# ludoplex/llamafile

Measured on AMD Instinct MI355X. Metric: prefill + decode tokens/sec, Llama-3-8B Q4_K_M, 1/2/4/8 MI355X vs CPU tinyBLAS, higher is better.
Workload: dtype int8; 1 GPU; llama3-8b-q4_k_m mat-muls (225 GGML_OP_MUL_MAT per pass, f32 activations in, quantisation fused, sibling ops fused at decode), 512-token prefill + 128 decode, matmul-only; model=llama3-8b-q4_k_m, parallelism=single GPU, hip_graph=True, weight_bytes_per_gpu=4616331264, decode_launches_per_pass=129

## Files before the change

### llamafile_amd/csrc/gemv_common.h

```cpp
#pragma once
#include "lfamd_device.h"
#include "gemv_launch.h"

__device__ static inline void load_piece(float (&v)[16], const float *x, int p) {
    const float4 *src = (const float4 *)(x + (size_t)p * 16);
#pragma unroll
    for (int e = 0; e < 4; e++) {
        float4 f = src[e];
        v[4 * e + 0] = f.x, v[4 * e + 1] = f.y, v[4 * e + 2] = f.z, v[4 * e + 3] = f.w;
    }
}

template <bool K, int N>
__device__ static inline void pack_codes(uint32_t (&y)[N / 4], const float (&v)[N], float scale) {
#pragma unroll
    for (int e = 0; e < N; e++) {
        int q;
        if constexpr (K) {
            q = (int)rintf(scale * v[e]);
            q = q > 127 ? 127 : q;
        } else {
            q = (int)roundf(v[e] * scale);
        }
        y[e >> 2] |= (uint32_t)(q & 0xff) << (8 * (e & 3));
    }
}

__device__ __forceinline__ void x80_quantise_piece(uint8_t *lds, int nquads, const float (&v)[16], int c, int p) {
    float amax = 0.0f;
#pragma unroll
    for (int e = 0; e < 16; e++)
        amax = fmaxf(amax, fabsf(v[e]));
    amax = fmaxf(amax, __shfl_xor(amax, 1, 64));
    const float d = amax / 127.0f;
    const float id = d != 0.0f ? 1.0f / d : 0.0f;
    uint32_t y[4] = {0, 0, 0, 0};
    pack_codes<false>(y, v, id);
    const int l = p >> 1, hf = p & 1;
    uint8_t *dst = lds + (size_t)(c * nquads + (l >> 2)) * X80_QUAD + (l & 3) * 4;
#pragma unroll
    for (int e = 0; e < 4; e++)
        *(uint32_t *)(dst + (4 * hf + e) * 16) = y[e];
    if (hf == 0)
        *(float *)(dst + X80_QD) = h2f(f2h_bits(d));
}
__device__ __forceinline__ void x80_copy_blocks(uint8_t *lds, int nquads, const uint8_t *__restrict__ B, size_t b_row_bytes, long col0, int nc,
                                                int nblocks, int nthr) {
    for (int idx = threadIdx.x; idx < nc * nblocks * 9; idx += nthr) {
        int c = idx / (nblocks * 9), rem = idx % (nblocks * 9);
        int l = rem / 9, w = rem % 9;
        const uint8_t *y = B + (col0 + c) * b_row_bytes + (size_t)l * 34;
        uint32_t v;
        if (w < 8) {
            const uint16_t *p = (const uint16_t *)(y + 2 + 4 * w);
            v = (uint32_t)p[0] | ((uint32_t)p[1] << 16);
        } else {
            v = __builtin_bit_cast(uint32_t, h2f(*(const uint16_t *)y));
        }
        *(uint32_t *)(lds + (size_t)(c * nquads + (l >> 2)) * X80_QUAD + (l & 3) * 4 + (w < 8 ? w * 16 : X80_QD)) = v;
    }
}

#ifndef GEMV_DIAG
#define GEMV_DIAG 0
#endif
#if GEMV_DIAG
#ifndef GEMV_DIAG_WG
#define GEMV_DIAG_WG 100
#endif
#define DIAG_STAMPS (4 * 16 * 16)
#include "diag_stamps.h"
static __device__ unsigned long long g_gemv_wg[512 * 4];
extern "C" __attribute__((weak)) int lfamd_debug_gemv_wgs(unsigned long long *dst) {
    return (int)hipMemcpyFromSymbol(dst, HIP_SYMBOL(g_gemv_wg), sizeof(g_gemv_wg));
}
#define GWG(slot)                                                                                                \
    do {                                                                                                         \
        if (blockIdx.x < 512 && threadIdx.x == 0) {                                                              \
            g_gemv_wg[blockIdx.x * 4 + (slot)] = __builtin_amdgcn_s_memrealtime();                               \
            if ((slot) == 0) {                                                                                   \
                g_gemv_wg[blockIdx.x * 4 + 2] = (unsigned long long)__builtin_amdgcn_s_getreg(4 | (31 << 11)) |  \
                                                ((unsigned long long)__builtin_amdgcn_s_getreg(20 | (31 << 11)) << 32); \
                gwg_clk0 = __builtin_amdgcn_s_memtime();                                                         \
            } else {  \
                g_gemv_wg[blockIdx.x * 4 + 3] = __builtin_amdgcn_s_memtime() - gwg_clk0;                         \
            }                                                                                                    \
        }                                                                                                        \
    } while (0)
#define GSTAMP()                                                                                                 \
    do {                                                                                                         \
        __builtin_amdgcn_sched_barrier(0);                                                                       \
        if ((blockIdx.x == 0 || blockIdx.x == GEMV_DIAG_WG) && lane == 0 && stamp_n < 16)                                  \
            g_stamps[((blockIdx.x ? 1 : 0) * 16 + wave) * 16 + stamp_n++] = DIAG_REALTIME();                      \
        __builtin_amdgcn_sched_barrier(0);                                                                       \
    } while (0)
#define GSTAMP_ARRIVAL()                                                                                         \
    do {                                                                                                         \
        asm volatile("s_waitcnt vmcnt(0)" ::: "memory");                                                         \
        GSTAMP();                                                                                                \
    } while (0)
#else
#define GSTAMP()
#define GSTAMP_ARRIVAL()
#define GWG(slot)
#endif
```

### llamafile_amd/csrc/gemv_impl.h

```cpp
#pragma once
#include "gemv_common.h"


__device__ static inline int put_group(uint8_t *dst, int grp, uint32_t y0, uint32_t y1) {
    const uint32_t p0 = __builtin_amdgcn_perm(y1, y0, 0x05010400);
    const uint32_t p1 = __builtin_amdgcn_perm(y1, y0, 0x07030602);
    const int pos = (grp & 16) | ((grp & 1) << 3) | ((grp & 8) >> 1) | ((grp >> 1) & 3);
    *(uint2 *)(dst + 8 * pos) = make_uint2(p0, p1);
    int hs = sdot4(y0, 0x01010101u, 0);
    hs = sdot4(y1, 0x01010101u, hs);
    *(int16_t *)(dst + XBLK_HB + 2 * pos) = (int16_t)hs;
    return hs;
}

__device__ static inline void put_pair(uint8_t *dst, int grp, int hs_even_plus_odd) {
    const int pp = ((grp & 16) >> 1) | ((grp & 1) << 2) | ((grp & 8) >> 2) | ((grp >> 2) & 1);
    *(int16_t *)(dst + XBLK_PS + 2 * pp) = (int16_t)hs_even_plus_odd;
}

__device__ static inline int put_group_pair(uint8_t *dst, int grp, uint32_t y0, uint32_t y1) {
    const int hs = put_group(dst, grp, y0, y1);
    const int pair = hs + (int)dpp_u32<DPP_XOR2>((uint32_t)hs);
    if ((grp & 2) == 0)
        put_pair(dst, grp, pair);
// ... 420 lines not shown
    struct chunk {
        uint4 q0[GEMV_CH_MAX], q1[GEMV_CH_MAX];
        uint2 hd[GEMV_CH_MAX], hm[GEMV_CH_MAX], hq[GEMV_CH_MAX];
    };
    __device__ static inline void load(chunk &ch, int s, lfamd_rsrc r, uint32_t off, int gsel, int slot, int hrow) {
        ch.q0[s] = buf_ld16_nt(r, off + (2 * gsel + 0) * 1024 + slot * 16);
        ch.q1[s] = buf_ld16_nt(r, off + (2 * gsel + 1) * 1024 + slot * 16);
        ch.hd[s] = buf_ld8(r, off + PCL_D + hrow * 16 + gsel * 8);
        if constexpr (HAS_M)
            ch.hm[s] = buf_ld8(r, off + PCL_M + hrow * 16 + gsel * 8);
        if constexpr (HAS_H)
            ch.hq[s] = buf_ld8(r, off + PCL_QH + slot * 16 + gsel * 8);
    }
    __device__ static inline float dot(const chunk &ch, int s, const uint8_t *xb, int gsel, int h) {
        const uint4 q0 = ch.q0[s], q1 = ch.q1[s];
        const uint2 hd = ch.hd[s];
        const kq_words8 qw = kq_words_of(q0, q1);
        const kq_codes y = kq_codes_of(xb, gsel, h);
        const uint4 dsw = *(const uint4 *)(xb + XBLK_D + 16 * gsel);
        const uint32_t dsv[4] = {dsw.x, dsw.y, dsw.z, dsw.w};
        kq_sums4 ps = {};
        if constexpr (!HAS_M)
            ps = kq_pair_sums_of(xb, gsel, h);
        float acc = 0.0f;
#pragma unroll
        for (int jj = 0; jj < 4; jj++) {
            int isum = 0;
#pragma unroll
            for (int d2 = 0; d2 < 2; d2++) {
                const int t8 = 2 * jj + d2;
                const uint32_t x = qw.w[t8];
                uint32_t c0 = x & 0x0F0F0F0F, c1 = (x >> 4) & 0x0F0F0F0F;
                if constexpr (HAS_H) {
                    const uint32_t Hd = (t8 < 4 ? ch.hq[s].x : ch.hq[s].y) >> (t8 & 3);
                    c0 |= Hd & 0x10101010;
                    c1 |= ((Hd >> 4) & 0x00100010) | ((Hd << 12) & 0x10001000);
                }
                isum = sdot4(c0, y.w[2 * t8], isum);
                isum = sdot4(c1, y.w[2 * t8 + 1], isum);
            }
            const float d = kq_h4(hd, jj);
            if constexpr (HAS_M) {
                const float m = kq_h4(ch.hm[s], jj);
                const float d8 = h2f((uint16_t)(dsv[jj] & 0xffff)), s8 = h2f((uint16_t)(dsv[jj] >> 16));
                acc = fmaf(d * d8, (float)isum, acc);
                acc = fmaf(m, h ? 0.0f : s8, acc);
            } else {
                acc = fmaf(d * __builtin_bit_cast(float, dsv[jj]), (float)(isum - 16 * ps.v[jj]), acc);
            }
        }
        return acc;
    }
};

template <int TYPE>
struct pk_traits {
    static constexpr int ACT = LFAMD_TYPE_Q8_K;
    static constexpr bool Q3 = TYPE == LFAMD_TYPE_Q3_K;
    static constexpr int TILE = Q3 ? PK3_TILE : PK2_TILE;
    static constexpr bool MINS = !Q3;
    static constexpr int OFF = Q3 ? 4 : 0;
    struct chunk {
        uint4 q[GEMV_CH_MAX];
        uint2 hb[GEMV_CH_MAX], sc[GEMV_CH_MAX];
        uint32_t dd[GEMV_CH_MAX];
    };
    __device__ static inline void load(chunk &ch, int s, lfamd_rsrc r, uint32_t off, int gsel, int slot, int hrow) {
        ch.q[s] = buf_ld16_nt(r, off + gsel * 1024 + slot * 16);
        if constexpr (Q3)
            ch.hb[s] = buf_ld8(r, off + PK3_HB + gsel * 512 + slot * 8);
        ch.sc[s] = buf_ld8(r, off + (Q3 ? PK3_SC : PK2_SC) + hrow * 16 + gsel * 8);
        ch.dd[s] = __builtin_amdgcn_raw_buffer_load_b32(r, off + (Q3 ? PK3_D : PK2_D) + hrow * 4, 0, 0);
    }
    __device__ static inline float dot(const chunk &ch, int s, const uint8_t *xb, int gsel, int h) {
        const uint4 qc = ch.q[s];
        const uint2 scb = ch.sc[s];
        const uint32_t dw = ch.dd[s];
        const float d = h2f((uint16_t)(dw & 0xffff));
        const uint32_t cw[4] = {qc.x, qc.y, qc.z, qc.w};
        const kq_codes y = kq_codes_of(xb, gsel, h);
        const kq_words4 hbv = kq_group_sums_of(xb, gsel, h);
        int sumi = 0, summ = 0;
#pragma unroll
        for (int t8 = 0; t8 < 8; t8++) {
            uint32_t x = ((t8 & 1) ? (cw[t8 >> 1] >> 2) : cw[t8 >> 1]) & 0x33333333u;
            if constexpr (Q3) {
                const uint32_t H = (t8 < 4 ? ch.hb[s].x : ch.hb[s].y) >> (t8 & 3);
                x |= (H & 0x11111111u) << 2;
            }
            const int isum = kq_nib_dot(x, y, t8, 0);
            const int hs = (int)(int16_t)((hbv.w[t8 >> 1] >> (16 * (t8 & 1))) & 0xffff);
            const uint32_t sbyte = ((t8 < 4 ? scb.x : scb.y) >> (8 * (t8 & 3))) & 0xff;
            if constexpr (Q3) {
                sumi += (int)(int8_t)sbyte * (isum - OFF * hs);
            } else {
                sumi += (int)(sbyte & 15) * isum;
                summ += (int)(sbyte >> 4) * hs;
            }
        }
        const float d8 = *(const float *)(xb + XBLK_D);
        if constexpr (MINS)
            return fmaf(d * d8, (float)sumi, -(h2f((uint16_t)(dw >> 16)) * d8) * (float)summ);
        return (d * d8) * (float)sumi;
    }
};

struct iq4c_traits {
    static constexpr int ACT = LFAMD_TYPE_Q8_K;
    static constexpr int TILE = P4K_TILE;
    struct chunk {
        uint4 q0[GEMV_CH_MAX], q1[GEMV_CH_MAX], hd[GEMV_CH_MAX];
    };
    __device__ static inline void load(chunk &ch, int s, lfamd_rsrc r, uint32_t off, int gsel, int slot, int hrow) {
        ch.q0[s] = buf_ld16_nt(r, off + (2 * gsel + 0) * 1024 + slot * 16);
        ch.q1[s] = buf_ld16_nt(r, off + (2 * gsel + 1) * 1024 + slot * 16);
        ch.hd[s] = buf_ld16(r, off + P4K_HDR + hrow * 16);
    }
    __device__ static inline float dot(const chunk &ch, int s, const uint8_t *xb, int gsel, int h) {
        const uint4 q0 = ch.q0[s], q1 = ch.q1[s], hd = ch.hd[s];
        const kq_words8 qw = kq_words_of(q0, q1);
        const kq_codes y = kq_codes_of(xb, gsel, h);
        const uint32_t scw = gsel ? hd.y : hd.x;
        int sumi = 0;
#pragma unroll
        for (int u = 0; u < 4; u++) {
            int isum = 0;
#pragma unroll
            for (int e = 0; e < 2; e++) {
                isum = kq_nib_dot<true>(qw.w[2 * u + e], y, 2 * u + e, isum);
            }
            sumi += (int)(int8_t)((scw >> (8 * u)) & 0xff) * isum;
        }
        const float d8 = *(const float *)(xb + XBLK_D);
        return (h2f((uint16_t)(hd.z & 0xffff)) * d8) * (float)sumi;
    }
};



__device__ static inline void put_codes_wave(uint8_t *dst, uint32_t y, int lane) {
    const int hf = lane & 1, grp = lane >> 1;
    const uint32_t other = dpp_u32<DPP_XOR1>(y);
    const uint32_t lo = hf ? other : y, hi = hf ? y : other;
    const uint32_t word = hf ? __builtin_amdgcn_perm(hi, lo, 0x07030602) : __builtin_amdgcn_perm(hi, lo, 0x05010400);
    const int pos = (grp & 16) | ((grp & 1) << 3) | ((grp & 8) >> 1) | ((grp >> 1) & 3);
    *(uint32_t *)(dst + 8 * pos + 4 * hf) = word;
    const int s4 = sdot4(y, 0x01010101u, 0);
    const int hs = s4 + (int)dpp_u32<DPP_XOR1>((uint32_t)s4);
    if (hf == 0)
        *(int16_t *)(dst + XBLK_HB + 2 * pos) = (int16_t)hs;
    const int hs2 = hs + (int)dpp_u32<DPP_ROW_SHL4>((uint32_t)hs);
    if ((lane & 5) == 0)
        put_pair(dst, grp, hs2);
}

__device__ static inline void stage_f32_q8k_wave(uint8_t *dst, const float4 v, int lane) {
    const float a0 = fabsf(v.x), a1 = fabsf(v.y), a2 = fabsf(v.z), a3 = fabsf(v.w);
    float am = fmaxf(fmaxf(a0, a1), fmaxf(a2, a3));
    am = fmaxf(am, dpp_f32<DPP_XOR1>(am));
    am = fmaxf(am, dpp_f32<DPP_XOR2>(am));
    am = fmaxf(am, dpp_f32<DPP_HALF_MIRROR>(am));
    am = fmaxf(am, dpp_f32<DPP_MIRROR>(am));
    const float amax = fmaxf(fmaxf(readlane_f32(am, 0), readlane_f32(am, 16)), fmaxf(readlane_f32(am, 32), readlane_f32(am, 48)));
    const bool m0 = a0 == amax, m1 = a1 == amax, m2 = a2 == amax, m3 = a3 == amax;
    const unsigned long long ball = __builtin_amdgcn_ballot_w64(m0 || m1 || m2 || m3);
    const float cand = m0 ? v.x : (m1 ? v.y : (m2 ? v.z : v.w));
    const int first = ball ? __builtin_ctzll(ball) : 0;
    const bool nz = amax != 0.0f;
    const float val = nz ? readlane_f32(cand, first) : 1.0f;
    const float iscale = -128.0f / val;
    int q0 = (int)rintf(iscale * v.x), q1 = (int)rintf(iscale * v.y), q2 = (int)rintf(iscale * v.z), q3 = (int)rintf(iscale * v.w);
    q0 = q0 > 127 ? 127 : q0, q1 = q1 > 127 ? 127 : q1, q2 = q2 > 127 ? 127 : q2, q3 = q3 > 127 ? 127 : q3;
    uint32_t y = (uint32_t)(q0 & 0xff) | ((uint32_t)(q1 & 0xff) << 8) | ((uint32_t)(q2 & 0xff) << 16) | ((uint32_t)(q3 & 0xff) << 24);
    y = nz ? y : 0u;
    const float d = nz ? 1.0f / iscale : 0.0f;
    put_codes_wave(dst, y, lane);
    if (lane == 0)
        *(float *)(dst + XBLK_D) = d;
}

template <bool S1>
__device__ static inline void stage_f32_q80_wave(uint8_t *dst, const float4 v, int lane) {
    float am = fmaxf(fmaxf(fabsf(v.x), fabsf(v.y)), fmaxf(fabsf(v.z), fabsf(v.w)));
    am = fmaxf(am, dpp_f32<DPP_XOR1>(am));
    am = fmaxf(am, dpp_f32<DPP_XOR2>(am));
    am = fmaxf(am, dpp_f32<DPP_HALF_MIRROR>(am));
    const float d = am / 127.0f;
    const float id = d != 0.0f ? 1.0f / d : 0.0f;
    const int q0 = (int)roundf(v.x * id), q1 = (int)roundf(v.y * id), q2 = (int)roundf(v.z * id), q3 = (int)roundf(v.w * id);
    const uint32_t y = (uint32_t)(q0 & 0xff) | ((uint32_t)(q1 & 0xff) << 8) | ((uint32_t)(q2 & 0xff) << 16) | ((uint32_t)(q3 & 0xff) << 24);
    put_codes_wave(dst, y, lane);
    int sum = 0;
    if constexpr (S1) {
        sum = sdot4(y, 0x01010101u, 0);
        sum += (int)dpp_u32<DPP_XOR1>((uint32_t)sum);
        sum += (int)dpp_u32<DPP_XOR2>((uint32_t)sum);
        sum += (int)dpp_u32<DPP_HALF_MIRROR>((uint32_t)sum);
    }
    if ((lane & 7) == 0)
        put_scale_q80<S1>(dst, lane >> 3, d, sum);
}

__device__ static inline void stage_f32_q8k_wave2(uint8_t *dst, const float4 va, const float4 vb, int lane) {
    const float v[8] = {va.x, va.y, va.z, va.w, vb.x, vb.y, vb.z, vb.w};
    float a[8];
#pragma unroll
    for (int e = 0; e < 8; e++)
        a[e] = fabsf(v[e]);
    float am = fmaxf(fmaxf(fmaxf(a[0], a[1]), fmaxf(a[2], a[3])), fmaxf(fmaxf(a[4], a[5]), fmaxf(a[6], a[7])));
    am = fmaxf(am, dpp_f32<DPP_XOR1>(am));
    am = fmaxf(am, dpp_f32<DPP_XOR2>(am));
    am = fmaxf(am, dpp_f32<DPP_HALF_MIRROR>(am));
    am = fmaxf(am, dpp_f32<DPP_MIRROR>(am));
    const bool hi = lane >= 32;
    const float amax_lo = fmaxf(readlane_f32(am, 0), readlane_f32(am, 16)), amax_hi = fmaxf(readlane_f32(am, 32), readlane_f32(am, 48));
    const float amax = hi ? amax_hi : amax_lo;
    bool any = false;
    float cand = v[7];
#pragma unroll
    for (int e = 7; e >= 0; e--) {
        const bool me = a[e] == amax;
        cand = me ? v[e] : cand;
        any = any || me;
    }
    const unsigned long long ball = __builtin_amdgcn_ballot_w64(any);
    const uint32_t blo = (uint32_t)ball, bhi = (uint32_t)(ball >> 32);
    const int first_lo = blo ? __builtin_ctz(blo) : 0, first_hi = 32 + (bhi ? __builtin_ctz(bhi) : 0);
    const float val_lo = readlane_f32(cand, first_lo), val_hi = readlane_f32(cand, first_hi);
    const bool nz = amax != 0.0f;
    const float val = nz ? (hi ? val_hi : val_lo) : 1.0f;
    const float iscale = -128.0f / val;
    uint32_t y[2] = {0, 0};
    pack_codes<true>(y, v, iscale);
    const uint32_t y0 = nz ? y[0] : 0u, y1 = nz ? y[1] : 0u;
    const float d = nz ? 1.0f / iscale : 0.0f;
    const int grp = lane & 31;
    put_group_pair(dst, grp, y0, y1);
    if (grp == 0)
        *(float *)(dst + XBLK_D) = d;
}

template <bool S1>
__device__ static inline void stage_f32_q80_wave2(uint8_t *dst, const float4 va, const float4 vb, int lane) {
    const float v[8] = {va.x, va.y, va.z, va.w, vb.x, vb.y, vb.z, vb.w};
    float am = 0.0f;
#pragma unroll
    for (int e = 0; e < 8; e++)
        am = fmaxf(am, fabsf(v[e]));
    am = fmaxf(am, dpp_f32<DPP_XOR1>(am));
    am = fmaxf(am, dpp_f32<DPP_XOR2>(am));
    const float d = am / 127.0f;
    const float id = d != 0.0f ? 1.0f / d : 0.0f;
    uint32_t y[2] = {0, 0};
    pack_codes<false>(y, v, id);
    const int grp = lane & 31;
    const int pair = put_group_pair(dst, grp, y[0], y[1]);
    const int sum = pair + (int)dpp_u32<DPP_XOR1>((uint32_t)pair);
    if ((grp & 3) == 0)
        put_scale_q80<S1>(dst, grp >> 2, d, sum);
}

template <int ACT, bool TAIL = false>
__device__ static inline void stage_quantised_wave(uint8_t *dst, const uint8_t *row_generic, int b, int lane, int kb = 0) {
    typedef const __attribute__((address_space(1))) uint8_t *gptr;
    const gptr row = (gptr)row_generic;
    if (lane < 32) {
        const int grp = lane;
        uint32_t y0, y1;
        if constexpr (ACT == LFAMD_TYPE_Q8_K) {
            const gptr y = row + (size_t)b * 292;
            const __attribute__((address_space(1))) uint32_t *src = (const __attribute__((address_space(1))) uint32_t *)(y + 36 + 8 * grp);
            y0 = src[0], y1 = src[1];
            if (grp == 0)
                *(float *)(dst + XBLK_D) = *(const __attribute__((address_space(1))) float *)y;
        } else {
            constexpr bool S1 = ACT == LFAMD_TYPE_Q8_1;
            const gptr blk = row + (size_t)(b * 8 + (grp >> 2)) * (S1 ? 36 : 34);
            const bool in = !TAIL || b * 8 + (grp >> 2) < kb;
            y0 = y1 = 0;
            if (in) {
                const __attribute__((address_space(1))) uint16_t *src = (const __attribute__((address_space(1))) uint16_t *)(blk + (S1 ? 4 : 2) + 8 * (grp & 3));
                y0 = (uint32_t)src[0] | ((uint32_t)src[1] << 16), y1 = (uint32_t)src[2] | ((uint32_t)src[3] << 16);
            }
            if ((grp & 3) == 0) {
                const __attribute__((address_space(1))) uint16_t *hdr = (const __attribute__((address_space(1))) uint16_t *)blk;
                if constexpr (S1)
                    *(uint32_t *)(dst + XBLK_D + 4 * (grp >> 2)) = in ? (uint32_t)hdr[0] | ((uint32_t)hdr[1] << 16) : 0u;
                else
                    *(float *)(dst + XBLK_D + 4 * (grp >> 2)) = in ? h2f(hdr[0]) : 0.0f;
            }
        }
        put_group_pair(dst, grp, y0, y1);
    }
}

#define KQ_F4(u) make_float4(__builtin_bit_cast(float, (u).x), __builtin_bit_cast(float, (u).y), __builtin_bit_cast(float, (u).z), \
                           __builtin_bit_cast(float, (u).w))

template <typename TR>
__device__ __forceinline__ int kq_nb_of(int nbk) {
    if constexpr (TR::ACT == LFAMD_TYPE_Q8_K)
        return nbk;
    else
        return (nbk + 7) >> 3;
}
template <typename TR>
__device__ __forceinline__ uint32_t kq_row_bytes_f32(int nbk) {
    return (uint32_t)nbk * (TR::ACT == LFAMD_TYPE_Q8_K ? 1024u : 128u);
}

template <typename TR, int NC, int BT, int NW, int GEMV_CH, bool IDS>
__device__ __forceinline__ void gemv_kq_body(const gemv_mats &mats, const int nbk, const uint8_t *__restrict__ B, size_t b_row_bytes,
                                             long col0, int n_ht, const int bid, const int gdim, uint8_t *lds) {
    const int nb = kq_nb_of<TR>(nbk), kb = nbk;
    const int lane = threadIdx.x & 63, wave = threadIdx.x >> 6;
    const int i16 = lane & 15, h = (lane >> 4) & 1, gsel = lane >> 5;
    const kq_lds lay = kq_lds_of(NC, nb, NW, 16);
    float *red = (float *)(lds + lay.red);
#if GEMV_DIAG
    int stamp_n = 0;
#endif
    GSTAMP();

    const int sb_per_wave = (nb + NW - 1) / NW;
    const int cpt = (sb_per_wave + GEMV_CH - 1) / GEMV_CH;
    const int ntile = (n_ht - bid + gdim - 1) / gdim;
    const int total = ntile * cpt;

    const int wave_u = __builtin_amdgcn_readfirstlane(wave);
    const uint32_t rt_bytes = (uint32_t)nb * TR::TILE;
    auto mat_of = [&](long ht) __attribute__((always_inline)) {
        int j = 0;
#pragma unroll
        for (int jj = 1; jj < GEMV_MAX_MATS; jj++)
            if (jj < mats.count && ht >= mats.ht_end[jj - 1])
                j = jj;
        return j;
    };
    auto issue = [&](typename TR::chunk &ch, int f) {
        const int tile_i = f / cpt, chunk_i = f - tile_i * cpt;
        long ht = (long)bid + (long)tile_i * gdim;
        const int j = mat_of(ht);
        const uint8_t *A = mats.A[j];
        bool have = f < total;
        if constexpr (IDS) {
            const int ex = mats.ids[mats.id_idx[j]];
            const bool ok = ex >= 0 && ex < mats.experts;
            A += (size_t)(ok ? ex : 0) * mats.expert_bytes;
            have = have && ok;
        }
        if (j > 0)
            ht -= mats.ht_end[j - 1];
        const int hh = (int)(ht & 1);
        const lfamd_rsrc r = make_rsrc(A + (size_t)(ht >> 1) * rt_bytes, have ? rt_bytes : 0u);
        const int slot = h * 32 + hh * 16 + i16, hrow = hh * 16 + i16;
#pragma unroll
        for (int s = 0; s < GEMV_CH; s++) {
            const int b = wave_u + NW * (chunk_i * GEMV_CH + s);
            TR::load(ch, s, r, (uint32_t)b * TR::TILE, gsel, slot, hrow);
        }
    };

    float acc[NC];
#pragma unroll
    for (int c = 0; c < NC; c++)
        acc[c] = 0.0f;

    auto consume = [&](const typename TR::chunk &ch, int f) {
        const int tile_i = f / cpt, chunk_i = f - tile_i * cpt;
#pragma unroll
        for (int s = 0; s < GEMV_CH; s++) {
            const int b = wave + NW * (chunk_i * GEMV_CH + s);
            const int bc = b < nb ? b : nb - 1;
#pragma unroll
            for (int c = 0; c < NC; c++) {
                acc[c] += TR::dot(ch, s, lds + (size_t)(c * nb + bc) * XBLK, gsel, h);
            }
        }
        if (chunk_i == cpt - 1) {
            float *rb = red + (tile_i & 1) * (NW * NC * 16);
#pragma unroll
            for (int c = 0; c < NC; c++) {
                float v = acc[c];
                v += __shfl_xor(v, 16, 64);
                v += __shfl_xor(v, 32, 64);
                if (lane < 16)
                    rb[(wave * NC + c) * 16 + lane] = v;
                acc[c] = 0.0f;
            }
            GSTAMP();
            __syncthreads();
            GSTAMP();
            if (threadIdx.x < 16 * NC) {
                const int c = threadIdx.x >> 4, i = threadIdx.x & 15;
                float v = 0.0f;
#pragma unroll
                for (int w = 0; w < NW; w++)
                    v += rb[(w * NC + c) * 16 + i];
                long ht = (long)bid + (long)tile_i * gdim;
                const int j = mat_of(ht);
                if (j > 0)
                    ht -= mats.ht_end[j - 1];
                const long row = (ht >> 1) * 32 + (ht & 1) * 16 + i;
// ... 148 lines not shown
struct kq_pre {
    const uint8_t *A0, *A1, *A2;
    int e0, e1;
};

template <typename TR, int BT, int NW, int GEMV_CH, bool IDS, bool EARLY = false, bool PAIR = false>
__device__ __forceinline__ void gemv_kq_body1(const gemv_mats &mats, int nbk, const uint8_t *__restrict__ B,
                                              size_t b_row_bytes, long col0, int n_ht, const int bid, int gdim,
                                              uint8_t *lds, const kq_pre pre) {
    if constexpr (EARLY)
        asm volatile("" : "+s"(nbk), "+s"(B), "+s"(n_ht), "+s"(gdim));
    else
        asm volatile("" : "+s"(nbk), "+s"(B), "+s"(b_row_bytes), "+s"(col0), "+s"(n_ht), "+s"(gdim));
    const int nb = kq_nb_of<TR>(nbk), kb = nbk;
    const int lane = threadIdx.x & 63;
    const int wave = __builtin_amdgcn_readfirstlane((int)(threadIdx.x >> 6));
    const int i16 = lane & 15, h = (lane >> 4) & 1, gsel = lane >> 5;
    constexpr int RW = PAIR ? 32 : 16;
    const kq_lds lay = kq_lds_of(1, nb, NW, RW);
    float *red = (float *)(lds + lay.red);
#if GEMV_DIAG
    int stamp_n = 0;
    unsigned long long gwg_clk0 = 0;
#endif
    GWG(0);
    GSTAMP();
    constexpr int JX = GEMV_CH == 1 ? 1 : (NW == 8 ? 2 : 4);
    const uint8_t *xrow = B + col0 * b_row_bytes;
    const lfamd_rsrc rx = make_rsrc(xrow, kq_row_bytes_f32<TR>(nbk));
    uint4 xv[JX];
    auto x_off = [&](int j0, int j) __attribute__((always_inline)) {
        if constexpr (JX == 1)
            return (uint32_t)(wave + NW * j0) * 1024u + (uint32_t)lane * 16u;
        else
            return (uint32_t)(wave + NW * (j0 + 2 * (j >> 1) + (lane >> 5))) * 1024u + (uint32_t)(lane & 31) * 32u + 16u * (j & 1);
    };
    if constexpr (BT == LFAMD_TYPE_F32) {
#pragma unroll
        for (int j = 0; j < JX; j++)
            xv[j] = buf_ld16(rx, x_off(0, j));
        __builtin_amdgcn_sched_barrier(0);
    }
    constexpr bool PRE1 = BT == LFAMD_TYPE_Q8_K && TR::ACT == LFAMD_TYPE_Q8_K && JX <= 2;
    uint2 pq = make_uint2(0, 0);
    uint32_t pd = 0;
    const int pre_b = JX == 1 ? wave : wave + NW * (lane >> 5);
    if constexpr (PRE1) {
        const lfamd_rsrc rq = make_rsrc(xrow, (uint32_t)nb * 292u);
        pq = buf_ld8(rq, (uint32_t)pre_b * 292u + 36u + (uint32_t)(lane & 31) * 8u);
        pd = __builtin_amdgcn_raw_buffer_load_b32(rq, (uint32_t)pre_b * 292u, 0, 0);
        __builtin_amdgcn_sched_barrier(0);
    }
    typename TR::chunk bufA, bufB;
    typename TR::chunk bufA2, bufB2;
    static_assert(!(PAIR && (EARLY || IDS)), "the paired item is a variant of the plain launch");
    constexpr bool early = EARLY && !IDS;
    constexpr bool XPAIR = !PAIR && TR::TILE % 128 != 0;
    auto ht_of = [&](int q) __attribute__((always_inline)) {
        return (XPAIR && q < (n_ht & ~15)) ? ((q & ~15) | ((q & 7) << 1) | ((q >> 3) & 1)) : q;
    };
    if constexpr (early) {
        const int hb = ht_of(bid);
        const bool s1 = hb >= pre.e0, s2 = hb >= pre.e1;
        const uint8_t *Ap = s2 ? pre.A2 : (s1 ? pre.A1 : pre.A0);
        const int hl = hb - (s2 ? pre.e1 : (s1 ? pre.e0 : 0));
        const int hh = hl & 1;
        const uint32_t rtb = (uint32_t)nb * TR::TILE;
        const lfamd_rsrc r = make_rsrc(Ap + (size_t)(hl >> 1) * rtb, hb < n_ht ? rtb : 0u);
#pragma unroll
        for (int s = 0; s < GEMV_CH; s++)
            TR::load(bufA, s, r, (uint32_t)(wave + NW * s) * TR::TILE, gsel, h * 32 + hh * 16 + i16, hh * 16 + i16);
        __builtin_amdgcn_sched_barrier(0);
        GSTAMP();
    }
    const kq_tab tab = kq_table(mats);

    const int sb_per_wave = (nb + NW - 1) / NW;
    const int cpt = (sb_per_wave + GEMV_CH - 1) / GEMV_CH;
    const uint32_t rt_bytes = (uint32_t)nb * TR::TILE;

    float acc = 0.0f, acc2 = 0.0f;
    int par = 0;
    constexpr int HT_STEP = PAIR ? 2 : 1;
    kq_cursor ci{HT_STEP * bid, 0}, cc{HT_STEP * bid, 0};
#define KQ_ADVANCE(c)                                                                                                  \
    do {                                                                                                               \
        if (++(c).chunk == cpt)                                                                                        \
            (c).chunk = 0, (c).ht += HT_STEP * gdim;                                                                   \
    } while (0)
#define KQ_ISSUE(buf)                                                                                                  \
    do {                                                                                                               \
        kq_issue<TR, NW, GEMV_CH, IDS>(buf, mats, tab, kq_cursor{ht_of(ci.ht), ci.chunk}, n_ht, rt_bytes, wave, i16, h, gsel); \
        if constexpr (PAIR) {                                                                                          \
            const kq_cursor c2{ci.ht + 1, ci.chunk};                                                                   \
            kq_issue<TR, NW, GEMV_CH, IDS>(buf##2, mats, tab, c2, n_ht, rt_bytes, wave, i16, h, gsel);                 \
        }                                                                                                              \
        KQ_ADVANCE(ci);                                                                                                \
    } while (0)
#define KQ_CONSUME(buf)                                                                                                \
    do {                                                                                                               \
        GSTAMP_ARRIVAL();                                                                                              \
        _Pragma("unroll") for (int s = 0; s < GEMV_CH; s++) {                                                          \
            const int b = wave + NW * (cc.chunk * GEMV_CH + s);                                                        \
                                                                        \
            if (b < nb) {                                                                                              \
                acc += TR::dot(buf, s, lds + (size_t)b * XBLK, gsel, h);                                               \
                if constexpr (PAIR)                                                                                    \
                    acc2 += TR::dot(buf##2, s, lds + (size_t)b * XBLK, gsel, h);                                       \
            }                                                                                                          \
        }                                                                                                              \
        if (cc.chunk == cpt - 1) {                                                                                     \
            float *rb = red + par * (NW * RW);                                                                         \
            par ^= 1;                                                                                                  \
            float v = kq_sum_rows(acc);                                   \
            if (lane < 16)                                                                                             \
                rb[wave * RW + lane] = v;                                                                              \
            acc = 0.0f;                                                                                                \
            if constexpr (PAIR) {                                                                                      \
                float v2 = kq_sum_rows(acc2);                                                                          \
                if (lane < 16)                                                                                         \
                    rb[wave * RW + 16 + lane] = v2;                                                                    \
                acc2 = 0.0f;                                                                                           \
            }                                                                                                          \
            GSTAMP();                                                                                                  \
            __syncthreads();                                                                                           \
            GSTAMP();                                                                                                  \
            if (threadIdx.x < RW) {                                                                                    \
                const int i = threadIdx.x;                                                                             \
                float t = 0.0f;                                                                                        \
                _Pragma("unroll") for (int w = 0; w < NW; w++) t += rb[w * RW + i];                                    \
                const kq_sel p = kq_pick(tab, ht_of(cc.ht));                                                           \
                const long row = (long)(p.ht >> 1) * 32 + (p.ht & 1) * 16 + i;          \
                bool ok = true;                                                                                        \
                if constexpr (IDS) {                    \
                    const int ex = mats.ids[p.idx];                                                                    \
                    ok = ex >= 0 && ex < mats.experts;                                                                 \
                }                                                                                                      \
                if (row < p.m && ok)                                                                                   \
                    ((__attribute__((address_space(1))) float *)p.C)[col0 * p.ldc + row] = t;                                                                      \
            }                                                                                                          \
        }                                                                                                              \
        KQ_ADVANCE(cc);                                                                                                \
    } while (0)

    if constexpr (BT == LFAMD_TYPE_F32) {
        uint8_t *dummy = (uint8_t *)(red + (lay.dummy - lay.red) / sizeof(float)) + (size_t)wave * XBLK;
        if constexpr (early)
            KQ_ADVANCE(ci);
        else
            KQ_ISSUE(bufA);
        __builtin_amdgcn_sched_barrier(0);
        GSTAMP();
#define KQ_STAGE_GROUP(j0)                                                                                             \
    if constexpr (JX == 1) {                                                                                           \
        const int b = wave + NW * (j0);                                                                                \
        uint8_t *dst = b < nb ? lds + (size_t)b * XBLK : dummy;                                                        \
        if constexpr (TR::ACT == LFAMD_TYPE_Q8_K)                                                                      \
            stage_f32_q8k_wave(dst, KQ_F4(xv[0]), lane);                                                               \
        else                                                                                                           \
            stage_f32_q80_wave<TR::ACT == LFAMD_TYPE_Q8_1>(dst, KQ_F4(xv[0]), lane);                                   \
    } else {                                                                                                           \
        _Pragma("unroll") for (int ps = 0; ps < JX / 2; ps++) {                                                        \
            const int b = wave + NW * ((j0) + 2 * ps + (lane >> 5));                                                   \
            uint8_t *dst = b < nb ? lds + (size_t)b * XBLK : dummy;                                                    \
            if constexpr (TR::ACT == LFAMD_TYPE_Q8_K)                                                                  \
                stage_f32_q8k_wave2(dst, KQ_F4(xv[2 * ps]), KQ_F4(xv[2 * ps + 1]), lane);                              \
            else                                                                                                       \
                stage_f32_q80_wave2<TR::ACT == LFAMD_TYPE_Q8_1>(dst, KQ_F4(xv[2 * ps]), KQ_F4(xv[2 * ps + 1]), lane);  \
        }                                                                                                              \
    }
        KQ_STAGE_GROUP(0)
        for (int j0 = JX; j0 < sb_per_wave; j0 += JX) {
#pragma unroll
            for (int j = 0; j < JX; j++)
                xv[j] = buf_ld16(rx, x_off(j0, j));
            KQ_STAGE_GROUP(j0)
        }
#undef KQ_STAGE_GROUP
    } else {
        if constexpr (early)
            KQ_ADVANCE(ci);
        else
            KQ_ISSUE(bufA);
        GSTAMP();
        if constexpr (PRE1 && JX == 1) {
            if (wave < nb && lane < 32) {
                uint8_t *dst = lds + (size_t)wave * XBLK;
                put_group_pair(dst, lane, pq.x, pq.y);
                if (lane == 0)
                    *(uint32_t *)(dst + XBLK_D) = pd;
            }
        } else if constexpr (PRE1) {
            {
                uint8_t *dummy = (uint8_t *)(red + (lay.dummy - lay.red) / sizeof(float)) + (size_t)wave * XBLK;
                uint8_t *dst = pre_b < nb ? lds + (size_t)pre_b * XBLK : dummy;
                const int grp = lane & 31;
                put_group_pair(dst, grp, pq.x, pq.y);
                if (grp == 0)
                    *(uint32_t *)(dst + XBLK_D) = pd;
            }
            for (int b = wave + 2 * NW; b < nb; b += NW)
                stage_quantised_wave<TR::ACT>(lds + (size_t)b * XBLK, xrow, b, lane);
        } else {
            if (TR::ACT != LFAMD_TYPE_Q8_K && kb != 8 * nb) {
                for (int b = wave; b < nb; b += NW) {
                    if (b * 8 + 8 > kb)
                        stage_quantised_wave<TR::ACT, true>(lds + (size_t)b * XBLK, xrow, b, lane, kb);
                    else
                        stage_quantised_wave<TR::ACT>(lds + (size_t)b * XBLK, xrow, b, lane);
                }
            } else {
                for (int b = wave; b < nb; b += NW)
                    stage_quantised_wave<TR::ACT>(lds + (size_t)b * XBLK, xrow, b, lane);
            }
        }
    }
    __builtin_amdgcn_fence(__ATOMIC_RELEASE, "wavefront");
    GSTAMP();

    for (;;) {
        kq_cursor cn = cc;
        KQ_ADVANCE(cn);
        if (cn.ht >= n_ht)
            break;
        KQ_ISSUE(bufB);
        KQ_CONSUME(bufA);
        GSTAMP();
        KQ_ISSUE(bufA);
        KQ_CONSUME(bufB);
    }
    if (cc.ht < n_ht)
        KQ_CONSUME(bufA);
    GWG(1);
#undef KQ_ADVANCE
#undef KQ_ISSUE
#undef KQ_CONSUME
}

template <typename TR, int NC, int BT, int NW, int GEMV_CH, bool IDS = false, bool PAIR = false>
__global__ __launch_bounds__(NW * 64) void gemv_kq_kernel(const uint8_t *__restrict__ B, size_t b_row_bytes, long col0, int nbk,
                                                          int n_ht, int gdim, const gemv_mats mats) {
    extern __shared__ __attribute__((aligned(16))) uint8_t lds[];
    if constexpr (NC == 1)
        gemv_kq_body1<TR, BT, NW, GEMV_CH, IDS, false, PAIR>(mats, nbk, B, b_row_bytes, col0, n_ht, (int)blockIdx.x, gdim, lds, kq_pre{});
    else
        gemv_kq_body<TR, NC, BT, NW, GEMV_CH, IDS>(mats, nbk, B, b_row_bytes, col0, n_ht, (int)blockIdx.x, gdim, lds);
}

template <typename TR, int NC, int BT, int NW, int GEMV_CH>
__global__ __launch_bounds__(NW * 64) void gemv_kq_early_kernel(const uint8_t *__restrict__ xrow, const uint8_t *__restrict__ A0,
                                                                const uint8_t *__restrict__ A1, const uint8_t *__restrict__ A2, int nbk,
                                                                int n_ht, int gdim, int e0, int e1, const gemv_mats mats) {
    extern __shared__ __attribute__((aligned(16))) uint8_t lds[];
    static_assert(NC == 1, "one activation row (the parameter keeps the kernel's name in line with gemv_kq_kernel's)");
    asm volatile("" : "+s"(A0), "+s"(A1), "+s"(A2), "+s"(e0), "+s"(e1));
    gemv_kq_body1<TR, BT, NW, GEMV_CH, false, true>(mats, nbk, xrow, 0, 0, n_ht, (int)blockIdx.x, gdim, lds, kq_pre{A0, A1, A2, e0, e1});
}

template <typename TR, int BT, int NW, int GEMV_CH>
__global__ __launch_bounds__(NW * 64) void gemv_kq_ids_pair_kernel(const uint8_t *__restrict__ Ba, const uint8_t *__restrict__ Bb,
                                                                   size_t b_row_bytes, int nbk, int n_ht_a, int n_ht_b, int grid_a, int grid_b,
                                                                   const gemv_mats mats_a, const gemv_mats mats_b) {
    extern __shared__ __attribute__((aligned(16))) uint8_t lds[];
    if ((int)blockIdx.x < grid_a)
        gemv_kq_body1<TR, BT, NW, GEMV_CH, true>(mats_a, nbk, Ba, b_row_bytes, 0, n_ht_a, (int)blockIdx.x, grid_a, lds, kq_pre{});
    else
        gemv_kq_body1<TR, BT, NW, GEMV_CH, true>(mats_b, nbk, Bb, b_row_bytes, 0, n_ht_b, (int)blockIdx.x - grid_a, grid_b, lds, kq_pre{});
}

template <typename TRA, typename TRB, int BT, int NW, int GEMV_CH>
__global__ __launch_bounds__(NW * 64) void gemv_kq_dual_kernel(const uint8_t *__restrict__ B, size_t b_row_bytes, int nbk, int n_ht_a,
                                                               int n_ht_b, int grid_a, int grid_b, const gemv_mats mats_a,
                                                               const gemv_mats mats_b) {
    extern __shared__ __attribute__((aligned(16))) uint8_t lds[];
    static_assert(TRA::ACT == TRB::ACT, "both types must share the activation image, and so the meaning of nbk (kq_nb_of)");
    if ((int)blockIdx.x < grid_a)
        gemv_kq_body1<TRA, BT, NW, GEMV_CH, false>(mats_a, nbk, B, b_row_bytes, 0, n_ht_a, (int)blockIdx.x, grid_a, lds, kq_pre{});
    else
        gemv_kq_body1<TRB, BT, NW, GEMV_CH, false>(mats_b, nbk, B, b_row_bytes, 0, n_ht_b, (int)blockIdx.x - grid_a, grid_b, lds, kq_pre{});
}

template <typename TRA, typename TRB, int BT, int NW, int GEMV_CH>
__global__ __launch_bounds__(NW * 64) void gemv_kq_dual_early_kernel(const uint8_t *__restrict__ xrow, const uint8_t *__restrict__ Aa0,
                                                                     const uint8_t *__restrict__ Aa1, const uint8_t *__restrict__ Ab0, int nbk,
                                                                     int n_ht_a, int n_ht_b, int grid_a, int ea0, int grid_b,
                                                                     const gemv_mats mats_a, const gemv_mats mats_b) {
    extern __shared__ __attribute__((aligned(16))) uint8_t lds[];
    static_assert(TRA::ACT == TRB::ACT, "both types must share the activation image, and so the meaning of nbk (kq_nb_of)");
    asm volatile("" : "+s"(Aa0), "+s"(Aa1), "+s"(Ab0), "+s"(ea0), "+s"(grid_a));
    if ((int)blockIdx.x < grid_a)
        gemv_kq_body1<TRA, BT, NW, GEMV_CH, false, true>(mats_a, nbk, xrow, 0, 0, n_ht_a, (int)blockIdx.x, grid_a, lds,
                                                         kq_pre{Aa0, Aa1, Aa1, ea0, KQ_NO_BOUNDARY});
    else
        gemv_kq_body1<TRB, BT, NW, GEMV_CH, false, true>(mats_b, nbk, xrow, 0, 0, n_ht_b, (int)blockIdx.x - grid_a, grid_b, lds,
                                                         kq_pre{Ab0, Ab0, Ab0, KQ_NO_BOUNDARY, KQ_NO_BOUNDARY});
}


template <typename TR, int BT, bool ROWS32>
static const void *kq_kernel_1(int variant, int nw, int ch) {
    const int form = nw * 10 + ch;
    if (variant == LFAMD_GEMV_PLAIN)
        return form == 82    ? (const void *)gemv_kq_kernel<TR, 1, BT, 8, 2>
               : form == 161 ? (const void *)gemv_kq_kernel<TR, 1, BT, 16, 1>
               : form == 162 ? (const void *)gemv_kq_kernel<TR, 1, BT, 16, 2>
                             : nullptr;
    if (variant == LFAMD_GEMV_EARLY)
        return form == 82    ? (const void *)gemv_kq_early_kernel<TR, 1, BT, 8, 2>
               : form == 161 ? (const void *)gemv_kq_early_kernel<TR, 1, BT, 16, 1>
               : form == 162 ? (const void *)gemv_kq_early_kernel<TR, 1, BT, 16, 2>
                             : nullptr;
    if constexpr (ROWS32)
        if (variant == LFAMD_GEMV_ROWS32 && form == 161)
            return (const void *)gemv_kq_kernel<TR, 1, BT, 16, 1, false, true>;
    return nullptr;
}

template <typename TR, int BT, int NC>
static const void *kq_kernel_n(int nw, int ch) {
    const int form = nw * 10 + ch;
    return form == 161  ? (const void *)gemv_kq_kernel<TR, NC, BT, 16, 1>
           : form == 82 ? (const void *)gemv_kq_kernel<TR, NC, BT, 8, 2>
           : form == 84 ? (const void *)gemv_kq_kernel<TR, NC, BT, 8, 4>
                        : nullptr;
}

template <typename TR, int BT, bool ROWS32>
static const void *kq_kernel(int variant, int nc, int nw, int ch) {
    static const void *(*const cols[])(int, int) = {kq_kernel_n<TR, BT, 2>, kq_kernel_n<TR, BT, 3>, kq_kernel_n<TR, BT, 4>, kq_kernel_n<TR, BT, 5>,
// ... 47 lines not shown
```

Before: 4456 tokens/s.

## Interleave f32 activation staging with weight-chunk pipeline and cheapen quantisation math

Replaces float abs-max reductions with integer-bit max via v_max3 and integer DPP compares, and replaces per-element int conversion and shift packing with a magic-number rounding trick plus byte permutes. The JX>1 f32 staging path is restructured so that activation loads and quantisation passes alternate with weight-buffer issue/consume steps (double buffering bufA/bufB) instead of staging everything up front. It also makes the diagnostic vmcnt wait conditional. The aim is to overlap activation quantisation with weight streaming and shorten the ALU path. In exchange the control flow is more complex, it adds an early-return path, and it relies on assumptions about chunk layout (GEMV_CH==2).

```diff
diff --git a/llamafile_amd/csrc/gemv_common.h b/llamafile_amd/csrc/gemv_common.h
--- a/llamafile_amd/csrc/gemv_common.h
+++ b/llamafile_amd/csrc/gemv_common.h
@@ -11,18 +11,23 @@
     }
 }
 
+#define KQ_ROUND_MAGIC 12582912.0f
 template <bool K, int N>
 __device__ static inline void pack_codes(uint32_t (&y)[N / 4], const float (&v)[N], float scale) {
+    uint32_t t[N];
 #pragma unroll
     for (int e = 0; e < N; e++) {
-        int q;
-        if constexpr (K) {
-            q = (int)rintf(scale * v[e]);
-            q = q > 127 ? 127 : q;
-        } else {
-            q = (int)roundf(v[e] * scale);
-        }
-        y[e >> 2] |= (uint32_t)(q & 0xff) << (8 * (e & 3));
+        float r;
+        if constexpr (K)
+            r = fminf(scale * v[e] + KQ_ROUND_MAGIC, KQ_ROUND_MAGIC + 127.0f);
+        else
+            r = roundf(v[e] * scale) + KQ_ROUND_MAGIC;
+        t[e] = __builtin_bit_cast(uint32_t, r);
+    }
+#pragma unroll
+    for (int e = 0; e < N; e += 4) {
+        const uint32_t lo = __builtin_amdgcn_perm(t[e + 1], t[e], 0x0c0c0400), hi = __builtin_amdgcn_perm(t[e + 3], t[e + 2], 0x0c0c0400);
+        y[e >> 2] |= __builtin_amdgcn_perm(hi, lo, 0x05040100);
     }
 }
 
@@ -96,7 +101,8 @@
     } while (0)
 #define GSTAMP_ARRIVAL()                                                                                         \
     do {                                                                                                         \
-        asm volatile("s_waitcnt vmcnt(0)" ::: "memory");                                                         \
+        if (GEMV_DIAG >= 2)                                                                                      \
+            asm volatile("s_waitcnt vmcnt(0)" ::: "memory");                                                     \
         GSTAMP();                                                                                                \
     } while (0)
 #else
diff --git a/llamafile_amd/csrc/gemv_impl.h b/llamafile_amd/csrc/gemv_impl.h
--- a/llamafile_amd/csrc/gemv_impl.h
+++ b/llamafile_amd/csrc/gemv_impl.h
@@ -596,6 +596,20 @@
     const int hs2 = hs + (int)dpp_u32<DPP_ROW_SHL4>((uint32_t)hs);
     if ((lane & 5) == 0)
         put_pair(dst, grp, hs2);
+}
+
+__device__ static inline uint32_t kq_absmax8_bits(const float (&v)[8]) {
+    float p, q, r;
+    asm("v_max3_f32 %0, |%1|, |%2|, |%3|" : "=v"(p) : "v"(v[0]), "v"(v[1]), "v"(v[2]));
+    asm("v_max3_f32 %0, |%1|, |%2|, |%3|" : "=v"(q) : "v"(v[3]), "v"(v[4]), "v"(v[5]));
+    asm("v_max3_f32 %0, |%1|, |%2|, %3" : "=v"(r) : "v"(v[6]), "v"(v[7]), "v"(p));
+    const uint32_t qb = __builtin_bit_cast(uint32_t, q), rb = __builtin_bit_cast(uint32_t, r);
+    return qb > rb ? qb : rb;
+}
+template <int CTRL>
+__device__ static inline uint32_t kq_max_dpp(uint32_t x) {
+    const uint32_t o = dpp_u32<CTRL>(x);
+    return o > x ? o : x;
 }
 
 __device__ static inline void stage_f32_q8k_wave(uint8_t *dst, const float4 v, int lane) {
@@ -647,31 +661,26 @@
 
 __device__ static inline void stage_f32_q8k_wave2(uint8_t *dst, const float4 va, const float4 vb, int lane) {
     const float v[8] = {va.x, va.y, va.z, va.w, vb.x, vb.y, vb.z, vb.w};
-    float a[8];
-#pragma unroll
-    for (int e = 0; e < 8; e++)
-        a[e] = fabsf(v[e]);
-    float am = fmaxf(fmaxf(fmaxf(a[0], a[1]), fmaxf(a[2], a[3])), fmaxf(fmaxf(a[4], a[5]), fmaxf(a[6], a[7])));
-    am = fmaxf(am, dpp_f32<DPP_XOR1>(am));
-    am = fmaxf(am, dpp_f32<DPP_XOR2>(am));
-    am = fmaxf(am, dpp_f32<DPP_HALF_MIRROR>(am));
-    am = fmaxf(am, dpp_f32<DPP_MIRROR>(am));
+    const uint32_t lm = kq_absmax8_bits(v);
+    uint32_t am = kq_max_dpp<DPP_XOR1>(lm);
+    am = kq_max_dpp<DPP_XOR2>(am);
+    am = kq_max_dpp<DPP_HALF_MIRROR>(am);
+    am = kq_max_dpp<DPP_MIRROR>(am);
     const bool hi = lane >= 32;
-    const float amax_lo = fmaxf(readlane_f32(am, 0), readlane_f32(am, 16)), amax_hi = fmaxf(readlane_f32(am, 32), readlane_f32(am, 48));
-    const float amax = hi ? amax_hi : amax_lo;
-    bool any = false;
+    const uint32_t r0 = (uint32_t)__builtin_amdgcn_readlane((int)am, 0), r1 = (uint32_t)__builtin_amdgcn_readlane((int)am, 16);
+    const uint32_t r2 = (uint32_t)__builtin_amdgcn_readlane((int)am, 32), r3 = (uint32_t)__builtin_amdgcn_readlane((int)am, 48);
+    const uint32_t amax_lo = r0 > r1 ? r0 : r1, amax_hi = r2 > r3 ? r2 : r3;
+    const uint32_t amax_b = hi ? amax_hi : amax_lo;
+    const float amax = __builtin_bit_cast(float, amax_b);
     float cand = v[7];
 #pragma unroll
-    for (int e = 7; e >= 0; e--) {
-        const bool me = a[e] == amax;
-        cand = me ? v[e] : cand;
-        any = any || me;
-    }
-    const unsigned long long ball = __builtin_amdgcn_ballot_w64(any);
-    const uint32_t blo = (uint32_t)ball, bhi = (uint32_t)(ball >> 32);
-    const int first_lo = blo ? __builtin_ctz(blo) : 0, first_hi = 32 + (bhi ? __builtin_ctz(bhi) : 0);
+    for (int e = 6; e >= 0; e--)
+        cand = fabsf(v[e]) == amax ? v[e] : cand;
+    const unsigned long long ball = __builtin_amdgcn_ballot_w64(lm == amax_b);
+    const uint32_t blo = (uint32_t)ball | 0x80000000u, bhi = (uint32_t)(ball >> 32) | 0x80000000u;
+    const int first_lo = __builtin_ctz(blo), first_hi = 32 + __builtin_ctz(bhi);
     const float val_lo = readlane_f32(cand, first_lo), val_hi = readlane_f32(cand, first_hi);
-    const bool nz = amax != 0.0f;
+    const bool nz = amax_b != 0u;
     const float val = nz ? (hi ? val_hi : val_lo) : 1.0f;
     const float iscale = -128.0f / val;
     uint32_t y[2] = {0, 0};
@@ -687,12 +696,10 @@
 template <bool S1>
 __device__ static inline void stage_f32_q80_wave2(uint8_t *dst, const float4 va, const float4 vb, int lane) {
     const float v[8] = {va.x, va.y, va.z, va.w, vb.x, vb.y, vb.z, vb.w};
-    float am = 0.0f;
-#pragma unroll
-    for (int e = 0; e < 8; e++)
-        am = fmaxf(am, fabsf(v[e]));
-    am = fmaxf(am, dpp_f32<DPP_XOR1>(am));
-    am = fmaxf(am, dpp_f32<DPP_XOR2>(am));
+    uint32_t amb = kq_absmax8_bits(v);
+    amb = kq_max_dpp<DPP_XOR1>(amb);
+    amb = kq_max_dpp<DPP_XOR2>(amb);
+    const float am = __builtin_bit_cast(float, amb);
     const float d = am / 127.0f;
     const float id = d != 0.0f ? 1.0f / d : 0.0f;
     uint32_t y[2] = {0, 0};
@@ -1147,29 +1154,69 @@
         __builtin_amdgcn_sched_barrier(0);
         GSTAMP();
 #define KQ_STAGE_GROUP(j0)                                                                                             \
-    if constexpr (JX == 1) {                                                                                           \
+    {                                                                                                                  \
         const int b = wave + NW * (j0);                                                                                \
         uint8_t *dst = b < nb ? lds + (size_t)b * XBLK : dummy;                                                        \
         if constexpr (TR::ACT == LFAMD_TYPE_Q8_K)                                                                      \
             stage_f32_q8k_wave(dst, KQ_F4(xv[0]), lane);                                                               \
         else                                                                                                           \
             stage_f32_q80_wave<TR::ACT == LFAMD_TYPE_Q8_1>(dst, KQ_F4(xv[0]), lane);                                   \
-    } else {                                                                                                           \
-        _Pragma("unroll") for (int ps = 0; ps < JX / 2; ps++) {                                                        \
-            const int b = wave + NW * ((j0) + 2 * ps + (lane >> 5));                                                   \
-            uint8_t *dst = b < nb ? lds + (size_t)b * XBLK : dummy;                                                    \
-            if constexpr (TR::ACT == LFAMD_TYPE_Q8_K)                                                                  \
-                stage_f32_q8k_wave2(dst, KQ_F4(xv[2 * ps]), KQ_F4(xv[2 * ps + 1]), lane);                              \
-            else                                                                                                       \
-                stage_f32_q80_wave2<TR::ACT == LFAMD_TYPE_Q8_1>(dst, KQ_F4(xv[2 * ps]), KQ_F4(xv[2 * ps + 1]), lane);  \
-        }                                                                                                              \
-    }
-        KQ_STAGE_GROUP(0)
-        for (int j0 = JX; j0 < sb_per_wave; j0 += JX) {
-#pragma unroll
-            for (int j = 0; j < JX; j++)
-                xv[j] = buf_ld16(rx, x_off(j0, j));
-            KQ_STAGE_GROUP(j0)
+    }
+        if constexpr (JX == 1) {
+            KQ_STAGE_GROUP(0)
+            for (int j0 = JX; j0 < sb_per_wave; j0 += JX) {
+                xv[0] = buf_ld16(rx, x_off(j0, 0));
+                KQ_STAGE_GROUP(j0)
+            }
+        } else {
+            static_assert(GEMV_CH == 2 && (JX == 2 || JX == 4), "a pass of two blocks is a chunk of two slots");
+#define KQ_LOAD_PASS(s0, xa, xb)                                                                                       \
+    do {                                                                                                               \
+        const uint32_t o = (uint32_t)(wave + NW * ((s0) + (lane >> 5))) * 1024u + (uint32_t)(lane & 31) * 32u;         \
+        xa = buf_ld16(rx, o), xb = buf_ld16(rx, o + 16u);                                                              \
+    } while (0)
+#define KQ_STAGE_PASS(s0, xa, xb)                                                                                      \
+    do {                                                                                                               \
+        const int b = wave + NW * ((s0) + (lane >> 5));                                                                \
+        uint8_t *dst = b < nb ? lds + (size_t)b * XBLK : dummy;                                                        \
+        if constexpr (TR::ACT == LFAMD_TYPE_Q8_K)                                                                      \
+            stage_f32_q8k_wave2(dst, KQ_F4(xa), KQ_F4(xb), lane);                                                      \
+        else                                                                                                           \
+            stage_f32_q80_wave2<TR::ACT == LFAMD_TYPE_Q8_1>(dst, KQ_F4(xa), KQ_F4(xb), lane);                          \
+        __builtin_amdgcn_fence(__ATOMIC_RELEASE, "wavefront");             \
+        GSTAMP();                                                                                                      \
+    } while (0)
+            constexpr int X1 = JX == 4 ? 2 : 0;
+            KQ_STAGE_PASS(0, xv[0], xv[1]);
+            if (cpt > 1) {
+                if constexpr (JX == 2)
+                    KQ_LOAD_PASS(2, xv[0], xv[1]);
+                KQ_ISSUE(bufB);
+                GSTAMP();
+                KQ_CONSUME(bufA);
+                KQ_STAGE_PASS(2, xv[X1], xv[X1 + 1]);
+                for (int c = 2; c < cpt; c += 2) {
+                    KQ_LOAD_PASS(2 * c, xv[0], xv[1]);
+                    if constexpr (JX == 4)
+                        KQ_LOAD_PASS(2 * c + 2, xv[2], xv[3]);
+                    KQ_ISSUE(bufA);
+                    KQ_CONSUME(bufB);
+                    KQ_STAGE_PASS(2 * c, xv[0], xv[1]);
+                    if constexpr (JX == 2)
+                        KQ_LOAD_PASS(2 * c + 2, xv[0], xv[1]);
+                    KQ_ISSUE(bufB);
+                    KQ_CONSUME(bufA);
+                    KQ_STAGE_PASS(2 * c + 2, xv[X1], xv[X1 + 1]);
+                }
+                KQ_ISSUE(bufA);
+                if (cc.ht >= n_ht) {
+                    GWG(1);
+                    return;
+                }
+                KQ_CONSUME(bufB);
+            }
+#undef KQ_LOAD_PASS
+#undef KQ_STAGE_PASS
         }
 #undef KQ_STAGE_GROUP
     } else {
```

Result: no change. 4460 tokens/s (median of 6 runs) (+0.1%).
